# TruongKhang/cds-mvsnet

Hardware: AMD Instinct MI355X
Metric: depth-maps/sec per ref view at 640x512 N=5 D=192 (single-stage plane sweep incl. CostRegNet + regression) (higher is better)
Workload: dtype f32; 1 GPU; M1: single-stage StageNet volume 640x512, D=192, C=8, N=5 views; parallelism=single

## Files before the change

cds_mvsnet_amd/_lib.py:

```python
from __future__ import annotations

import ctypes
import os
from ctypes import c_float, c_int, c_longlong, c_void_p

_HERE = os.path.dirname(os.path.abspath(__file__))
LIB_PATH = os.environ.get("CDS_MVSNET_LIB") or os.path.join(_HERE, "libcdsmvs_hip.so")

ACT_NONE, ACT_RELU, ACT_LEAKY01, ACT_SIGMOID, ACT_TANH = 0, 1, 2, 3, 4
ACT_ACCUM = 16
AGG_ACCUMULATE, AGG_NORMALIZE, AGG_CHANNELS_LAST, AGG_FAST_POSITIONS = 1, 2, 4, 8
WARP_FAST_POSITIONS = AGG_FAST_POSITIONS
MAX_VIEWS = 8
MAX_IMAGES = 16
STAGE_STATE_WORDS = 2080
DEPTH_METRICS_MAX_T = 8
DEPTH_METRICS_MAX_GROUPS = 1024
ICP_SUMS = 18
ICP_MAX_GROUPS = 1024
CROP_MAX_VERTICES = 256
RANSAC_RECORD = 15
RANSAC_MIN_SAMPLE, RANSAC_MAX_SAMPLE = 3, 8
EINVAL = -1000

# ... 13 lines not shown
    "cds_warp_aggregate_f32": [P, P, P, P, P, P, P, I, I, I, I, I, I, I, P],
    "cds_warp_entropy_window_f32": [P, P, P, P, P, I, I, I, I, I, I, I, I, P],
    "cds_warp_aggregate_window_f32": [P, P, P, P, P, P, P, I, I, I, I, I, I, I, I, P],
    "cds_warp_aggregate_bwd_f32": [P, P, P, P, P, P, P, P, P, I, I, I, I, I, I, P],
    "cds_volume_finish_f32": [P, P, P, I, I, I, I, P, P, P],
    "cds_volume_finish_bwd_f32": [P, P, P, P, P, I, I, I, I, P, P, P, P, P],
    "cds_volume_normalize_f32": [P, P, I, I, I, P],
    "cds_volume_normalize_cl_f32": [P, P, I, I, I, P],
    "cds_softargmin_conf_f32": [P, P, P, P, P, I, I, I, I, P],
    "cds_depth_hypotheses_f32": [P, P, I, I, I, I, I, I, P, P, P],
    "cds_depth_planes_f32": [P, I, I, I, P, P],
    "cds_conv3d_k3_f32": [P, P, P, P, P, I, I, I, I, I, I, I, P],
    "cds_conv3d_k3_cl_f32": [P, P, P, P, P, I, I, I, I, I, I, P],
    "cds_conv3d_sbf_f32": [P, P, P, P, P, I, I, I, I, I, I, I, P],
    "cds_conv3d_sf16_f32": [P, P, P, P, I, I, I, I, I, I, I, P, F, P, P],
    "cds_deconv3d_sbf_f32": [P, P, P, P, P, I, I, I, I, I, I, I, P],
    "cds_deconv3d_sf16_f32": [P, P, P, P, P, I, I, I, I, I, I, P, F, P, P],
    "cds_deconv3d_zm_sf16_f32": [P, P, P, P, P, I, I, I, I, I, I, P, F, P, P],
    "cds_deconv_prob_zm_f32": [P, P, P, P, P, P, I, I, I, P],
    "cds_deconv_prob_zm_sf16_f32": [P, P, P, P, P, P, I, I, I, P, F, P],
    "cds_deconv_prob_zm_sf16_mfma_f32": [P, P, P, P, P, P, P, I, I, I, P, F, P, F, F, P],
    "cds_deconv3d_zm_f32": [P, P, P, P, P, I, I, I, I, I, I, P],
    "cds_deconv3d_k3s2_f32": [P, P, P, P, P, I, I, I, I, I, I, P],
    "cds_conv2d_f32": [P, P, P, P, I, I, I, I, I, I, I, I, I, P],
    "cds_conv2d_affine_f32": [P, P, P, P, P, I, I, I, I, I, I, I, I, I, P],
    "cds_instnorm_affine_f32": [P, P, P, I, I, I, I, F, P],
    "cds_fpn_stats_parts": [I, I],
    "cds_conv2d_fpn_f32": [P, P, P, P, P, P, P, I, I, I, I, I, I, P],
    "cds_conv2d_k3_c16_f32": [P, P, P, P, P, P, I, I, I, I, P],
    "cds_dynconv_branches_sbf_f32": [P, P, P, P, P, I, I, I, I, I, P, I, P],
    "cds_dynconv_fused_sbf_f32": [P, P, P, P, P, P, P, P, F, P, P, P, I, I, I, I, I, P, I, P],
    "cds_dynconv_fused_parts": [I, I],
    "cds_conv2d_k3_relu_sbf_f32": [P, P, P, P, P, P, I, I, I, I, P],
    "cds_dynconv_blend_f32": [P, P, P, P, P, F, P, P, I, I, I, I, I, P],
    "cds_dynconv_blend_shared_f32": [P, P, P, P, P, F, P, P, I, I, I, I, I, I, P],
    "cds_blend_stats_parts": [I, I],
    "cds_dynconv_blend_stats_f32": [P, P, P, P, P, F, P, P, P, I, I, I, I, I, I, P],
    "cds_instnorm_reduce_f32": [P, I, P, P, I, I, I, I, F, P],
    "cds_instnorm_apply_f32": [P, P, P, I, I, I, I, I, I, P],
    "cds_instnorm_act_f32": [P, P, P, I, I, I, I, I, I, P],
    "cds_debug_poison_lds": [ctypes.c_uint],
    "cds_dynconv_cl_parts": [I, I],
    "cds_dynconv_cl_f32": [P, P, P, P, P, P, P, P, F, P, P, P, I, I, I, I, P, I, P],
    "cds_dynconv_cl_sf16_f32": [P, P, P, P, P, P, P, P, F, P, P, P, I, I, I, I, P, I, F, F, P],
    "cds_conv00_cl_f32": [P, P, P, P, P, P, P, F, P, P, P, I, I, I, I, P],
    "cds_conv00_cl_sf16_f32": [P, P, P, P, P, P, P, F, P, P, P, I, I, I, I, P, F, P],
    "cds_blend_cl_parts": [I, I],
    "cds_dynconv_blend_cl_f32": [P, P, P, P, P, F, P, P, P, I, I, I, I, I, I, P],
    "cds_conv2d_k3s2_cl_f32": [P, P, P, P, I, I, I, I, I, P],
    "cds_conv2d_k3s2_cl_sf16_f32": [P, P, P, P, I, I, I, I, I, F, F, P],
    "cds_fpn_cl_parts": [I, I],
    "cds_conv2d_fpn_cl_f32": [P, P, P, P, P, P, P, I, I, I, I, I, I, P],
    "cds_vis_layer1_cl_f32": [P, P, P, P, P, I, I, I, P],
    "cds_conv2d_k3_relu_cl_f32": [P, P, P, P, P, P, I, I, I, I, P],
    "cds_instnorm_stats_cl_parts": [I, I],
    "cds_instnorm_stats_cl_f32": [P, P, I, I, I, I, P],
    "cds_instnorm_apply_cl_f32": [P, P, P, P, I, I, I, I, I, I, I, P],
    "cds_curvature_stats_f32": [P, P, P, P, P, I, P],
    "cds_curvature_stats_bwd_f32": [P, P, P, P, P, P, P, P, I, P],
    "cds_pair_mean_f32": [P, P, I, I, P],
    "cds_view_mean_f32": [P, P, I, I, P],
    "cds_depth_affine_f32": [P, P, I, P, P],
    "cds_deconv2d_k3s2_f32": [P, P, P, P, I, I, I, I, I, P],
    "cds_refine_finish_f32": [P, P, P, I, I, P, P],
    "cds_bn3d_stats_f32": [P, P, I, I, L, P],
    "cds_bn3d_norm_f32": [P, P, P, P, DB, DB, F, P, P, P, P, P, P, P, P, I, I, L, I, P],
    "cds_bn3d_bwd_reduce_f32": [P, P, P, P, P, I, I, L, I, P],
    "cds_bn3d_bwd_norm_f32": [P, P, P, P, P, P, P, DB, P, P, P, I, I, L, I, P],
    "cds_conv3d_wgrad_f32": [P, P, P, I, I, I, I, I, I, I, I, I, I, P],
    "cds_bn3d_norm_bound_f32": [P, P, P, P, DB, DB, F, P, P, P, P, P, P, P, P, I, I, L, I, P, P],
    "cds_bn3d_bwd_norm_bound_f32": [P, P, P, P, P, P, P, DB, P, P, P, I, I, L, I, P, P],
    "cds_absmax_bound_f32": [P, L, P, P],
    "cds_sf16_pack_conv3d_f32": [P, P, P, P, I, I, I, P],
    "cds_conv3d_k3_sf16_f32": [P, P, P, P, P, I, I, I, I, I, I, I, P],
    "cds_conv3d_wgrad_sf16_f32": [P, P, P, P, P, I, I, I, I, I, I, I, I, I, I, P],
    "cds_conv2d_wgrad_f32": [P, P, P, I, I, I, I, I, I, I, I, I, I, P],
    "cds_conv2d_dgrad_s2_f32": [P, P, P, I, I, I, I, I, I, I, P],
    "cds_instnorm_bwd_f32": [P, P, P, P, P, I, I, I, I, I, I, P],
    "cds_dynconv_bn_stats_f32": [P, P, P, P, P, P, P, P, I, I, I, I, I, I, F, F, I, I, P],
    "cds_dynconv_blend_train_f32": [P, P, P, P, P, P, P, P, F, P, P, I, I, I, I, I, I, P],
    "cds_dynconv_blend_bwd_f32": [P, P, P, P, P, P, P, P, F, P, P, P, P, P, I, I, I, I, I, I, I, I, P],
    "cds_f32_to_bf16": [P, P, L, P],
    "cds_instnorm_act_b16_f32": [P, P, P, P, P, I, I, I, I, I, I, P],
    "cds_conv2d_wgrad_xb16_f32": [P, P, P, I, I, I, I, I, I, I, I, I, I, P],
    "cds_instnorm_bwd_yb16_f32": [P, P, P, P, P, P, I, I, I, I, I, I, P],
    "cds_dynconv_bn_stats_b16_f32": [P, P, P, P, P, P, P, P, I, I, I, I, I, I, F, F, I, I, P],
    "cds_dynconv_blend_train_b16_f32": [P, P, P, P, P, P, P, P, F, P, P, I, I, I, I, I, I, P],
    "cds_dynconv_blend_bwd_b16_f32": [P, P, P, P, P, P, P, P, F, P, P, P, P, P, I, I, I, I, I, I, I, I, P],
    "cds_pack_conv2d_f32": [P, P, P, P, I, I, I, I, P],
    "cds_pack_conv3d_f32": [P, P, P, I, I, I, P],
    "cds_softargmin_bwd_f32": [P, P, P, P, I, I, I, I, P],
    "cds_dynconv_bwd_finish_f32": [P, P, I, I, P, P],
    "cds_bn_running_update_f32": [P, P, P, F, I, I, P, P, P],
    "cds_loss_records": [ctypes.c_longlong],
    "cds_loss_stage_f32": [P, P, P, P, P, P, P, I, I, I, P, P, P],
    "cds_loss_final_f32": [P, P, P, P, P, P, I, P, P, P, P],
    "cds_loss_stage_bwd_f32": [P, P, P, P, P, P, P, P, F, I, I, I, P, P, P, P],
    "cds_feat_target_f32": [P, P, P, F, F, I, I, I, P, P],
    "cds_depth_fusion_f32": [P, P, P, P, P, P, P, P, P, I, I, I, P, F, F, F, P],
    "cds_depth_fusion_dynamic_f32": [P, P, P, P, P, P, P, P, P, P, I, I, I, P, F, F, I, I, P],
    "cds_depth_normals_f32": [P, P, P, I, I, I, F, I, P, P, P],
    "cds_voxel_merge_f32": [P, P, P, L, P, P, L, P, P, P, P, P],
    "cds_tsdf_integrate_f32": [P, L, P, P, DB, P, P, P, P, I, I, I, P, P, P, P, P],
    "cds_tsdf_integrate_w_f32": [P, L, P, P, DB, P, P, P, P, I, I, I, P, P, P, P, P, I, F, P, P],
    "cds_tsdf_view_weights": [P, P, P, P, P, P, I, I, P, P],
    "cds_tsdf_classify": [P, P, L, P, P, P, P, I, P, P, P, P, P],
# ... 89 lines not shown
```

cds_mvsnet_amd/csrc/feat_cl.hip:

```cpp
#include "sbf_common.hpp"
#include "feat_common.hpp"

namespace {

constexpr int TX = 32, TY = 8;

struct DynEpi {
  const float* w1;
  const float* b1;
  const float* w2;
  float* out;
  float* norm_curv;
  double* partial;
  float temperature;
  const float* epi;
  float xs, omul;
};

constexpr int cmax(int a, int b) { return a > b ? a : b; }
constexpr int nks_of(int k) { return (k * k + 3) / 4; }

template <int CIN, int K0, int K1, int K2, int MODE = 1>
struct DCfg {
  static constexpr int NBR = MODE == 2 ? 1 : (K2 > 0 ? 3 : 2);
// ... 1022 lines not shown
      const int ky = tap / 3, kx = tap - ky * 3;
      const unsigned char* ap = lp + ((2 * wave + ky) * IXP + 2 * m + kx) * POSB;
      BV wh[NBLK], wlo[NBLK], ah[2], alo[2];
#pragma unroll
      for (int nb = 0; nb < NBLK; ++nb) {
        const uint4* p = wr + (size_t)((t * NBLK + nb) * 3) * 64;
        wh[nb].u = p[0];
        wlo[nb].u = p[64];
      }
#pragma unroll
      for (int q = 0; q < 2; ++q) {
        const unsigned char* a = ap + q * 32 * POSB;
        ah[q].u = *reinterpret_cast<const uint4*>(a);
        alo[q].u = *reinterpret_cast<const uint4*>(a + 16);
      }
      __builtin_amdgcn_sched_barrier(0);
#pragma unroll
      for (int nb = 0; nb < NBLK; ++nb) {
#pragma unroll
        for (int q = 0; q < 2; ++q) SF16_MFMA(acc[nb][q], alo[q], wh[nb]);
#pragma unroll
        for (int q = 0; q < 2; ++q) SF16_MFMA(acc[nb][q], ah[q], wlo[nb]);
#pragma unroll
        for (int q = 0; q < 2; ++q) SF16_MFMA(acc[nb][q], ah[q], wh[nb]);
      }
    }
  }
  __syncthreads();
  float* trL = reinterpret_cast<float*>(lds) + wave * (2 * NBLK * 16 * C::TP);
#pragma unroll
  for (int nb = 0; nb < NBLK; ++nb)
#pragma unroll
    for (int q = 0; q < 2; ++q) {
      const f32x4 a = acc[nb][q] * omul;
      const float v[4] = {a.x, a.y, a.z, a.w};
#pragma unroll
      for (int i = 0; i < 4; ++i) trL[((q * NBLK + nb) * 16 + g * 4 + i) * C::TP + m] = v[i];
    }
  wave_lds_fence();
  const int oy = oy0 + wave;
  if (oy < Ho) {
#pragma unroll
    for (int q = 0; q < 2; ++q) {
      const int ox = ox0 + q * 16 + m;
      if (ox >= Wo) continue;
      float* __restrict__ op = out + (((size_t)img * Ho + oy) * Wo + ox) * COUT;
#pragma unroll
      for (int nb = 0; nb < NBLK; ++nb)
        *reinterpret_cast<float4*>(op + nb * 16 + 4 * g) = *reinterpret_cast<const float4*>(trL + ((q * NBLK + nb) * 16 + m) * C::TP + 4 * g);
    }
  }
}

}

extern "C" int cds_vis_layer1_cl_f32(const float* entropy, const float* ref_nc, const float* weight, const float* bias, float* out, int V,
                                     int H, int W, void* stream) {
  if (!entropy || !ref_nc || !weight || !bias || !out || V < 1 || H < 1 || W < 1) return CDS_EINVAL;
  hipLaunchKernelGGL(vis_layer1_cl_kernel, dim3(cds_ceil_div(H * W, 256), V), dim3(256), 0, (hipStream_t)stream, entropy, ref_nc, weight,
                     bias, out, H, W);
  return cds_launch_status();
}

extern "C" int cds_conv2d_k3_relu_cl_f32(const float* x, const void* weight_split, const float* bias, const float* head_w,
                                         const float* head_b, float* out, int N, int Cin, int H, int W, void* stream) {
  if (!x || !weight_split || !out || N < 1 || Cin != 16 || H < 1 || W < 1 || (head_w != nullptr) != (head_b != nullptr)) return CDS_EINVAL;
  DynEpi ep{};
  ep.w1 = head_w;
  ep.b1 = head_b;
  ep.out = out;
  return launch_dynconv_cl<16, 3, 0, 0, 2>(x, nullptr, weight_split, bias, ep, N, H, W, (hipStream_t)stream);
}

extern "C" int cds_dynconv_cl_parts(int H, int W) { return cds_ceil_div(W, TX) * cds_ceil_div(H, TY); }

extern "C" int cds_dynconv_cl_f32(const float* x, const float* in_affine, const void* weight_split, const float* bias,
                                  const float* w1, const float* b1, const float* w2, const float* epipoles, float temperature,
                                  float* out, float* norm_curv, double* partial, int N, int C, int H, int W, const int* ksizes, int nb,
                                  void* stream) {
  if (!x || !weight_split || !w1 || !b1 || !w2 || !epipoles || !out || !norm_curv || !partial || !ksizes || N < 1 ||
      N > CDS_MAX_IMAGES || H < 1 || W < 1 || nb < 2 || nb > 3)
    return CDS_EINVAL;
  DynEpi ep{};
  ep.w1 = w1; ep.b1 = b1; ep.w2 = w2; ep.out = out; ep.norm_curv = norm_curv; ep.partial = partial; ep.temperature = temperature;
  ep.epi = epipoles;
  hipStream_t st = (hipStream_t)stream;
  const int k0 = ksizes[0], k1 = ksizes[1], k2 = nb == 3 ? ksizes[2] : 0;
  if (C == 8 && k0 == 3 && k1 == 5 && k2 == 7) return launch_dynconv_cl<8, 3, 5, 7>(x, in_affine, weight_split, bias, ep, N, H, W, st);
  if (C == 8 && k0 == 1 && k1 == 3 && k2 == 0) return launch_dynconv_cl<8, 1, 3, 0>(x, in_affine, weight_split, bias, ep, N, H, W, st);
  if (C == 16 && k0 == 3 && k1 == 5 && k2 == 0) return launch_dynconv_cl<16, 3, 5, 0>(x, in_affine, weight_split, bias, ep, N, H, W, st);
  if (C == 16 && k0 == 1 && k1 == 3 && k2 == 0) return launch_dynconv_cl<16, 1, 3, 0>(x, in_affine, weight_split, bias, ep, N, H, W, st);
  if (C == 32 && k0 == 1 && k1 == 3 && k2 == 0) return launch_dynconv_cl<32, 1, 3, 0>(x, in_affine, weight_split, bias, ep, N, H, W, st);
  return CDS_EINVAL;
}

extern "C" int cds_dynconv_cl_sf16_f32(const float* x, const float* in_affine, const void* weight_split, const float* bias,
                                       const float* w1, const float* b1, const float* w2, const float* epipoles, float temperature,
                                       float* out, float* norm_curv, double* partial, int N, int C, int H, int W, const int* ksizes,
                                       int nb, float x_bound, float w_inv_scale, void* stream) {
  if (!x || !weight_split || !w1 || !b1 || !w2 || !epipoles || !out || !norm_curv || !partial || !ksizes || N < 1 ||
      N > CDS_MAX_IMAGES || H < 1 || W < 1 || nb < 2 || nb > 3 || !(x_bound > 0.f) || !(w_inv_scale > 0.f))
    return CDS_EINVAL;
  DynEpi ep{};
  ep.w1 = w1; ep.b1 = b1; ep.w2 = w2; ep.out = out; ep.norm_curv = norm_curv; ep.partial = partial; ep.temperature = temperature;
  ep.epi = epipoles;
  int e = 0;
  (void)frexpf(x_bound, &e);
  e = e > 100 ? 100 : (e < -100 ? -100 : e);
  ep.xs = ldexpf(1.0f, 15 - e);
  ep.omul = w_inv_scale / ep.xs;
  hipStream_t st = (hipStream_t)stream;
  const int k0 = ksizes[0], k1 = ksizes[1], k2 = nb == 3 ? ksizes[2] : 0;
  if (C == 8 && k0 == 3 && k1 == 5 && k2 == 7) return launch_dynconv_cl<8, 3, 5, 7, 1, true>(x, in_affine, weight_split, bias, ep, N, H, W, st);
  if (C == 8 && k0 == 1 && k1 == 3 && k2 == 0) return launch_dynconv_cl<8, 1, 3, 0, 1, true>(x, in_affine, weight_split, bias, ep, N, H, W, st);
  if (C == 16 && k0 == 3 && k1 == 5 && k2 == 0) return launch_dynconv_cl<16, 3, 5, 0, 1, true>(x, in_affine, weight_split, bias, ep, N, H, W, st);
  if (C == 16 && k0 == 1 && k1 == 3 && k2 == 0) return launch_dynconv_cl<16, 1, 3, 0, 1, true>(x, in_affine, weight_split, bias, ep, N, H, W, st);
  if (C == 32 && k0 == 1 && k1 == 3 && k2 == 0) return launch_dynconv_cl<32, 1, 3, 0, 1, true>(x, in_affine, weight_split, bias, ep, N, H, W, st);
  return CDS_EINVAL;
}

static int conv00_entry(const float* x, const void* weight_split, const float* bias, const float* w1, const float* b1, const float* w2,
                        const float* epipoles, float temperature, float* out, float* norm_curv, double* partial, int N, int n_shared,
                        int H, int W, const float* in_bound, float w_inv_scale, void* stream) {
  if (!x || !weight_split || !w1 || !b1 || !w2 || !epipoles || !out || !norm_curv || !partial || N < 1 || N > CDS_MAX_IMAGES ||
// ... 145 lines not shown
```

cds_mvsnet_amd/csrc/lib.hip:

```cpp
#include "cds_common.hpp"
extern "C" int cds_version(void) { return 100;  }

namespace {
__global__ __launch_bounds__(1024) void poison_lds_kernel(unsigned pattern, int words) {
  extern __shared__ unsigned lds_words[];
  for (int i = threadIdx.x; i < words; i += 1024) lds_words[i] = pattern;
}
}

extern "C" int cds_debug_poison_lds(unsigned pattern) {
  const int bytes = 160 * 1024;
  static std::atomic<unsigned long long> ok{0};
  if (int e = cds_allow_lds(reinterpret_cast<const void*>(poison_lds_kernel), bytes, ok)) return e;
  if (hipDeviceSynchronize() != hipSuccess) return -1;
  hipLaunchKernelGGL(poison_lds_kernel, dim3(2048), dim3(1024), bytes, 0, pattern, bytes / 4);
  if (hipDeviceSynchronize() != hipSuccess) return -1;
  return 0;
}
```

cds_mvsnet_amd/model.py:

```python
from __future__ import annotations

import os
import weakref
from typing import Dict, List, Optional, Sequence, Tuple

import torch
import torch.nn as nn
import torch.nn.functional as F

from . import geometry, ops
from .ops import ACT_LEAKY01, ACT_NONE, ACT_RELU, ACT_SIGMOID, ACT_TANH

Tensor = torch.Tensor
BN_EPS = 1e-5
USE_SPLIT_BF16 = os.environ.get("CDS_CONV_EXACT", "0") != "1"
USE_FUSED_BLEND = os.environ.get("CDS_FUSED_BLEND", "1") != "0"
OVERLAP_STAGE1 = os.environ.get("CDS_OVERLAP_STAGE1", "1") != "0"
OVERLAP_STAGE2 = os.environ.get("CDS_OVERLAP_STAGE2", "0") == "1"
USE_FEAT_CL = os.environ.get("CDS_FEAT_CL", "1") != "0"
USE_CONV00_MFMA = os.environ.get("CDS_CONV00_MFMA", "1") != "0"
OVERLAP_IN_CAPTURE = os.environ.get("CDS_OVERLAP_IN_CAPTURE", "1") != "0"
_SIDE_STREAMS: Dict[int, "torch.cuda.Stream"] = {}
USE_GRAPHS_DEFAULT = os.environ.get("CDS_GRAPH", "0") == "1"
_GRAPH_RUNNERS: "weakref.WeakKeyDictionary" = weakref.WeakKeyDictionary()


_UNIT_BOUNDS: Dict[int, Tensor] = {}


def _unit_bound(device) -> Tensor:
    idx = device.index if device.index is not None else torch.cuda.current_device()
    if idx not in _UNIT_BOUNDS:
        _UNIT_BOUNDS[idx] = torch.ones((1,), dtype=torch.float32, device=device)
    return _UNIT_BOUNDS[idx]


def _side_stream(device) -> "torch.cuda.Stream":
    idx = device.index if device.index is not None else torch.cuda.current_device()
    if idx not in _SIDE_STREAMS:
        _SIDE_STREAMS[idx] = torch.cuda.Stream(device=device)
    return _SIDE_STREAMS[idx]


def _bn_fold(bn: nn.Module) -> Tuple[Tensor, Tensor]:
    scale = bn.weight.detach() / torch.sqrt(bn.running_var + bn.eps)
    shift = bn.bias.detach() - bn.running_mean * scale
    return scale, shift


def _pack2d(w: Tensor) -> Tensor:
    cout, cin, k, _ = w.shape
    p = w.permute(1, 2, 3, 0).reshape(cin, k * k, cout)
    pad = (-cout) % 8
    if pad:
        p = F.pad(p, (0, pad))
    return p.contiguous()


class _Packed:

    def __init__(self):
        self._entries: Dict[object, Tuple[tuple, Dict[str, Tensor]]] = {}
        self.generation = 0

    def invalidate(self) -> None:
        self._entries = {}
        self.generation += 1

    @staticmethod
    def _tensors(owner: nn.Module) -> List[Tensor]:
        return list(owner.parameters()) + list(owner.buffers())

    def get(self, owner: nn.Module, builder) -> Dict[str, Tensor]:
# ... 534 lines not shown
            return self._conv00(x[0])
        p = self.p
        w, kw = self._operand(name, *x)
        return ops.dynconv_cl(x[0], w, p.get(f"{name}.bs"), dc.size_kernels, p[f"{name}.m1"], p[f"{name}.mb"], p[f"{name}.m2"],
                              self.epi[level], self.T, 0.1, in_affine=x[1], **kw)

    def down(self, name: str, x):
        w, kw = self._operand(name, *x, plain=".w9")
        y = ops.conv2d_k3s2_cl(x[0], None if kw else w, getattr(self.net, name).conv.out_channels, x[1], wsplit=w if kw else None, **kw)
        return y, ops.instnorm_stats_cl(y, 0.1)[1]

    def lateral(self, name: str, coarse, skip):
        return ops.conv2d_fpn_cl(coarse[0], skip[0], self.p[f"{name}.wt"], getattr(self.net, name).conv.out_channels, coarse[1], skip[1], 0.1)

    def head(self, name: str, x, level: int, stage: int):
        o, nc, st, _ = self._dynconv(name, getattr(self.net, name), x, level)
        n = self.n_chw
        if stage == 2:
            on, chw = ops.instnorm_apply_cl(o, st, ACT_TANH, n, cl_from=0)
            return (chw, on[n:] if n < o.shape[0] else None), (on, None), nc
        hwc, chw = ops.instnorm_apply_cl(o, st, ACT_TANH, n, cl_from=n)
        return (chw, hwc), None, nc


class StageNet(_PackedHolder):
    def __init__(self, num_mvs_stages: int = 3):
        super().__init__()
        self.vis = nn.ModuleList([nn.Sequential(ConvBn2d(2, 16), ConvBn2d(16, 16), ConvBn2d(16, 16),
                                                nn.Conv2d(16, 1, 1), nn.Sigmoid()) for _ in range(num_mvs_stages)])
        self._init_packed()

    def _pack(self) -> Dict[str, Tensor]:
        out: Dict[str, Tensor] = {}
        for s, seq in enumerate(self.vis):
            for i in range(3):
                scale, shift = _bn_fold(seq[i].bn)
                wf = seq[i].conv.weight.detach() * scale.view(-1, 1, 1, 1)
                out[f"{s}.w{i}"] = _pack2d(wf)
                out[f"{s}.b{i}"] = shift.contiguous()
                if i > 0:
                    out[f"{s}.wcl{i}"] = wf.permute(2, 3, 0, 1).reshape(9, 16, 16).contiguous()
                    if USE_SPLIT_BF16 and wf.is_cuda:
                        out[f"{s}.ws{i}"] = ops.split_pack_dynconv([wf])
            out[f"{s}.w3"] = _pack2d(seq[3].weight.detach())
            out[f"{s}.b3"] = seq[3].bias.detach().contiguous()
            out[f"{s}.hw"] = seq[3].weight.detach().reshape(16).contiguous()
        return out

    def visibility(self, entropy: Tensor, ref_nc: Tensor, stage_idx: int) -> Tensor:
        p = self._packed.get(self, self._pack)
        s = stage_idx
        with ops.prof("visibility_cnn"):
            if USE_FEAT_CL and f"{s}.ws1" in p and ops.USE_CONV2D_SBF:
                x = ops.vis_layer1_cl(entropy.contiguous(), ref_nc.contiguous(), p[f"{s}.w0"], p[f"{s}.b0"])
                x = ops.conv2d_k3_relu_cl(x, p[f"{s}.ws1"], p[f"{s}.b1"])
                return ops.conv2d_k3_relu_cl(x, p[f"{s}.ws2"], p[f"{s}.b2"], head_w=p[f"{s}.hw"], head_b=p[f"{s}.b3"])
            x = torch.stack((entropy, ref_nc), dim=1)
            x = ops.conv2d(x, p[f"{s}.w0"], p[f"{s}.b0"], 16, 3, 1, 1, ACT_RELU)
            if f"{s}.ws1" in p and ops.USE_CONV2D_SBF and x.shape[-1] % 4 == 0:
                x = ops.conv2d_k3_relu_sbf(x, p[f"{s}.ws1"], p[f"{s}.b1"])
                return ops.conv2d_k3_relu_sbf(x, p[f"{s}.ws2"], p[f"{s}.b2"], head_w=p[f"{s}.hw"], head_b=p[f"{s}.b3"])
            if ops.conv2d_c16_supported(x):
                x = ops.conv2d_k3_c16(x, p[f"{s}.wcl1"], p[f"{s}.b1"], ACT_RELU)
                return ops.conv2d_k3_c16(x, p[f"{s}.wcl2"], p[f"{s}.b2"], ACT_RELU, head_w=p[f"{s}.hw"], head_b=p[f"{s}.b3"])
            for i in (1, 2):
                x = ops.conv2d(x, p[f"{s}.w{i}"], p[f"{s}.b{i}"], 16, 3, 1, 1, ACT_RELU)
            return ops.conv2d(x, p[f"{s}.w3"], p[f"{s}.b3"], 1, 1, 1, 0, ACT_SIGMOID)[:, 0]

    def aggregate(self, ref_chw: Tensor, src_hwc: Tensor, ref_nc: Tensor, mats: Tensor, hyp: Tensor, stage_idx: int,
                  normalize: bool = True, channels_last: bool = False):
        ent = ops.warp_entropy(ref_chw, src_hwc, mats, hyp)
        vis = self.visibility(ent, ref_nc, stage_idx).contiguous()
        volume, vis_sum = ops.warp_aggregate(ref_chw, src_hwc, vis, mats, hyp, normalize=normalize, channels_last=channels_last)
        return volume, vis_sum, ent, vis

    def run_single(self, ref_chw, src_hwc, ref_nc, nc_sums, mats, hyp, cost_regularization, stage_idx, vol_bound=None, nc_mean=None):
        cl = isinstance(cost_regularization, CostRegNet) and cost_regularization.split_bf16_supported()
        volume, _, _, _ = self.aggregate(ref_chw, src_hwc, ref_nc, mats, hyp, stage_idx, channels_last=cl)
        if cl:
            if vol_bound is None and ops.USE_SPLIT_F16:
                vol_bound = (ref_chw.abs().amax() * src_hwc.abs().amax()).reshape(1)
            depth, conf = cost_regularization.regress(volume, hyp, bound=vol_bound)
        else:
            depth, conf = ops.softargmin_conf(cost_regularization(volume), hyp)
        del volume
        if nc_mean is None:
            nc_mean = ops.view_mean(nc_sums.contiguous())
        return depth, conf, nc_mean

    def forward(self, features, proj_matrices, depth_values, num_depth, cost_regularization, prob_volume_init=None,
                stage_idx=0, gt_depth=None):
        if prob_volume_init is not None:
            raise NotImplementedError("prob_volume_init is dead code in the reference (never passed)")
        assert len(features) == proj_matrices.shape[1] - 1, "Different number of images and projection matrices"
        assert depth_values.shape[1] == num_depth, f"depth_values.shape[1]:{depth_values.shape[1]}  num_depth:{num_depth}"
        if self.training or gt_depth is not None:
            from .training import stage_forward_train
            dv = depth_values
            if dv.dim() == 2:
                h, w = features[0]["ref"][0].shape[-2:]
                dv = dv.view(*dv.shape, 1, 1).expand(-1, -1, h, w)
            with torch.cuda.device(dv.device):
                return stage_forward_train(self, features, proj_matrices, dv, cost_regularization, stage_idx, gt_depth)
        with torch.cuda.device(depth_values.device):
            return self._forward(features, proj_matrices, depth_values, cost_regularization, stage_idx)

# ... 267 lines not shown
```

cds_mvsnet_amd/ops.py:

```python
from __future__ import annotations

import ctypes
import os
from typing import Optional, Tuple

import torch

from . import _lib
from ._lib import (ACT_LEAKY01, ACT_NONE, ACT_RELU, ACT_SIGMOID, ACT_TANH, AGG_ACCUMULATE, AGG_CHANNELS_LAST, AGG_FAST_POSITIONS,
                   AGG_NORMALIZE,
                   MAX_IMAGES, MAX_VIEWS, check)

Tensor = torch.Tensor

PROFILE_ON = False
PROFILE: dict = {}
PROFILE_HOST_MS: dict = {}


class prof:

    def __init__(self, name: str):
        self.name = name
        self.start = None
# ... 1100 lines not shown
    check(lib.cds_conv2d_fpn_cl_f32(_dev(coarse_cl, "coarse"), _dev(coarse_affine, "coarse_affine") if coarse_affine is not None else None,
                                    _dev(skip_cl, "skip"), _dev(skip_affine, "skip_affine") if skip_affine is not None else None,
                                    _dev(w, "weight"), out.data_ptr(), partial.data_ptr() if partial is not None else None,
                                    N, Ca, Cb, cout, H, W, _stream(skip_cl)), "cds_conv2d_fpn_cl_f32")
    if stats_slope is None:
        return out
    return out, _reduce_records(partial, N, cout, H, W, stats_slope)[1]


def instnorm_apply_cl(x_cl: Tensor, stats: Tensor, act: int, n_chw: int = 0, cl_from: Optional[int] = 0):
    N, H, W, C = x_cl.shape
    if stats.dtype != torch.float64 or tuple(stats.shape) != (N, C, 2):
        raise ValueError(f"instnorm_apply_cl: stats must be float64 [{N},{C},2]")
    want_cl = cl_from is not None and cl_from < N
    if not want_cl and n_chw < 1:
        raise ValueError("instnorm_apply_cl: nothing to write")
    dev = x_cl.device
    out_cl = torch.empty((N - cl_from, H, W, C), dtype=torch.float32, device=dev) if want_cl else None
    out_chw = torch.empty((n_chw, C, H, W), dtype=torch.float32, device=dev) if n_chw > 0 else None
    check(_lib.load().cds_instnorm_apply_cl_f32(_dev(x_cl, "x"), _dev64(stats, "stats"), out_cl.data_ptr() if want_cl else None,
                                                out_chw.data_ptr() if n_chw > 0 else None, N, C, H, W, act, n_chw,
                                                cl_from if want_cl else 0, _stream(x_cl)), "cds_instnorm_apply_cl_f32")
    return out_cl, out_chw


def vis_layer1_cl(entropy: Tensor, ref_nc: Tensor, wpk: Tensor, bias: Tensor) -> Tensor:
    V, h, w = entropy.shape
    if tuple(ref_nc.shape) != (V, h, w) or tuple(wpk.shape) != (2, 9, 16) or bias.numel() != 16:
        raise ValueError(f"vis_layer1_cl: need entropy / ref_nc [V,h,w], weight [2,9,16], bias [16]; got {tuple(entropy.shape)}, "
                         f"{tuple(ref_nc.shape)}, {tuple(wpk.shape)}")
    out = torch.empty((V, h, w, 16), dtype=torch.float32, device=entropy.device)
    check(_lib.load().cds_vis_layer1_cl_f32(_dev(entropy, "entropy"), _dev(ref_nc, "ref_nc"), _dev(wpk, "weight"), _dev(bias, "bias"),
                                            out.data_ptr(), V, h, w, _stream(entropy)), "cds_vis_layer1_cl_f32")
    return out


def conv2d_k3_relu_cl(x_cl: Tensor, wsplit: Tensor, bias: Optional[Tensor], head_w: Optional[Tensor] = None,
                      head_b: Optional[Tensor] = None) -> Tensor:
    N, H, W, C = x_cl.shape
    if C != 16:
        raise ValueError(f"conv2d_k3_relu_cl: need [N,H,W,16], got {tuple(x_cl.shape)}")
    if (head_w is None) != (head_b is None) or (head_w is not None and (head_w.numel() != 16 or head_b.numel() != 1)):
        raise ValueError("conv2d_k3_relu_cl: head_w [16] and head_b [1] go together")
    if wsplit.dtype != torch.int16 or wsplit.numel() != 2 * 3 * 1 * 3 * 64 * 8:
        raise ValueError("conv2d_k3_relu_cl: wsplit must be split_pack_dynconv([w]) of a [16,16,3,3] weight")
    out = torch.empty((N, H, W) if head_w is not None else (N, H, W, 16), dtype=torch.float32, device=x_cl.device)
    check(_lib.load().cds_conv2d_k3_relu_cl_f32(_dev(x_cl, "x"), wsplit.data_ptr(), _dev(bias, "bias") if bias is not None else None,
                                                _dev(head_w, "head_w") if head_w is not None else None,
                                                _dev(head_b, "head_b") if head_b is not None else None,
                                                out.data_ptr(), N, C, H, W, _stream(x_cl)), "cds_conv2d_k3_relu_cl_f32")
    return out


def depth_fusion(ref_depth: Tensor, ref_conf: Tensor, src_depths: Tensor, src_confs: Tensor, cams: Tensor,
                 prob_thresh, dist_thresh: float, depth_thresh: float, view_thresh: float,
                 want_view_masks: bool = False):
    V, h, w = src_depths.shape
    if tuple(ref_depth.shape) != (h, w) or tuple(ref_conf.shape) != (3, h, w) or tuple(src_confs.shape) != (V, 3, h, w) \
            or tuple(cams.shape) != (V, 100):
        raise ValueError("depth_fusion: inconsistent shapes")
    dev = ref_depth.device
    fused = torch.empty((h, w), dtype=torch.float32, device=dev)
    mask = torch.empty((h, w), dtype=torch.float32, device=dev)
    points = torch.empty((3, h, w), dtype=torch.float32, device=dev)
    vm = torch.empty((V, h, w), dtype=torch.float32, device=dev) if want_view_masks else None
    th = torch.tensor([float(p) for p in prob_thresh], dtype=torch.float32)
    if th.numel() != 3:
        raise ValueError("depth_fusion: three confidence thresholds expected")
    check(_lib.load().cds_depth_fusion_f32(_dev(ref_depth, "ref_depth"), _dev(ref_conf, "ref_conf"),
                                           _dev(src_depths, "src_depths"), _dev(src_confs, "src_confs"),
                                           _dev(cams, "cams"), fused.data_ptr(), mask.data_ptr(), points.data_ptr(),
                                           vm.data_ptr() if vm is not None else None, V, h, w, _host(th, "prob_thresh"),
                                           float(dist_thresh), float(depth_thresh), float(view_thresh),
                                           _stream(fused)), "cds_depth_fusion_f32")
    return fused, mask, points, vm


DYNAMIC_MAX_LEVELS = 16


def depth_fusion_dynamic(ref_depth: Tensor, ref_conf: Tensor, src_depths: Tensor, src_confs: Tensor, cams: Tensor,
                         prob_thresh, dist_base: float = 0.25, rel_base: float = 1.0 / 1300.0, n_views=(2, 10),
                         want_admit: bool = False, want_levels: bool = False):
    V, h, w = src_depths.shape
    if tuple(ref_depth.shape) != (h, w) or tuple(ref_conf.shape) != (3, h, w) or tuple(src_confs.shape) != (V, 3, h, w) \
            or tuple(cams.shape) != (V, 100):
        raise ValueError("depth_fusion_dynamic: inconsistent shapes")
    if len(n_views) != 2:
        raise ValueError(f"depth_fusion_dynamic: n_views must be (n_min, n_max), got {n_views!r}")
    n_min, n_max = int(n_views[0]), int(n_views[1])
    if n_min < 1 or n_max < n_min or n_max > DYNAMIC_MAX_LEVELS:
        raise ValueError(f"depth_fusion_dynamic: need 1 <= n_min <= n_max <= {DYNAMIC_MAX_LEVELS}, got {(n_min, n_max)}")
    if not (float(dist_base) > 0.0 and float(rel_base) > 0.0):
        raise ValueError(f"depth_fusion_dynamic: dist_base and rel_base must be positive, got {dist_base}, {rel_base}")
    th = torch.tensor([float(p) for p in prob_thresh], dtype=torch.float32)
    if th.numel() != 3:
        raise ValueError("depth_fusion_dynamic: three confidence thresholds expected")
    dev = ref_depth.device
    fused = torch.empty((h, w), dtype=torch.float32, device=dev)
    mask = torch.empty((h, w), dtype=torch.float32, device=dev)
    points = torch.empty((3, h, w), dtype=torch.float32, device=dev)
    admit = torch.empty((h, w), dtype=torch.uint8, device=dev) if want_admit else None
    levels = torch.empty((V, h, w), dtype=torch.uint8, device=dev) if want_levels else None
    check(_lib.load().cds_depth_fusion_dynamic_f32(_dev(ref_depth, "ref_depth"), _dev(ref_conf, "ref_conf"),
                                                   _dev(src_depths, "src_depths"), _dev(src_confs, "src_confs"),
                                                   _dev(cams, "cams"), fused.data_ptr(), mask.data_ptr(), points.data_ptr(),
# ... 449 lines not shown
```

include/cds_mvsnet_hip.h:

```cpp
#ifndef CDS_MVSNET_HIP_H
#define CDS_MVSNET_HIP_H

#ifdef __cplusplus
extern "C" {
#endif

#define CDS_EINVAL (-1000)
#define CDS_MAX_VIEWS 8
#define CDS_MAX_IMAGES 16
#define CDS_STAGE_STATE_WORDS 2080

#define CDS_ACT_NONE 0
#define CDS_ACT_RELU 1
#define CDS_ACT_LEAKY01 2
#define CDS_ACT_SIGMOID 3
#define CDS_ACT_ACCUM 16
#define CDS_ACT_TANH 4

#define CDS_AGG_ACCUMULATE 1
#define CDS_AGG_NORMALIZE 2
#define CDS_AGG_CHANNELS_LAST 4
#define CDS_AGG_FAST_POSITIONS 8
#define CDS_WARP_FAST_POSITIONS CDS_AGG_FAST_POSITIONS

// ... 117 lines not shown
int cds_dynconv_blend_shared_f32(const float* branches, const float* w1, const float* b1, const float* w2,
                                 const float* epipoles, float temperature, float* out, float* norm_curv, int N,
                                 int K, int Cout, int H, int W, int n_shared, void* stream);

int cds_blend_stats_parts(int H, int W);
int cds_dynconv_blend_stats_f32(const float* branches, const float* w1, const float* b1, const float* w2,
                                const float* epipoles, float temperature, float* out, float* norm_curv,
                                float* partial, int N, int K, int Cout, int H, int W, int n_shared, void* stream);
int cds_instnorm_reduce_f32(const float* partial, int parts, float* stats, float* affine, int N, int C, int H, int W,
                            float slope, void* stream);
int cds_instnorm_apply_f32(const float* x, const float* stats, float* out, int N, int C, int H, int W, int act,
                           int out_hwc, void* stream);

int cds_instnorm_act_f32(const float* x, float* out, float* stats, int N, int C, int H, int W, int act,
                         int out_hwc, void* stream);
int cds_instnorm_affine_f32(const float* x, float* affine, float* stats, int N, int C, int H, int W, float slope,
                            void* stream);

int cds_debug_poison_lds(unsigned pattern);

int cds_dynconv_cl_parts(int H, int W);
int cds_dynconv_cl_f32(const float* x, const float* in_affine, const void* weight_split, const float* bias, const float* w1,
                       const float* b1, const float* w2, const float* epipoles, float temperature, float* out,
                       float* norm_curv, double* partial, int N, int C, int H, int W, const int* ksizes, int nb, void* stream);
int cds_dynconv_cl_sf16_f32(const float* x, const float* in_affine, const void* weight_split, const float* bias, const float* w1,
                            const float* b1, const float* w2, const float* epipoles, float temperature, float* out, float* norm_curv,
                            double* partial, int N, int C, int H, int W, const int* ksizes, int nb, float x_bound, float w_inv_scale,
                            void* stream);

int cds_conv00_cl_f32(const float* x, const void* weight_split, const float* bias, const float* w1, const float* b1, const float* w2,
                      const float* epipoles, float temperature, float* out, float* norm_curv, double* partial, int N, int n_shared,
                      int H, int W, void* stream);
int cds_conv00_cl_sf16_f32(const float* x, const void* weight_split, const float* bias, const float* w1, const float* b1, const float* w2,
                           const float* epipoles, float temperature, float* out, float* norm_curv, double* partial, int N, int n_shared,
                           int H, int W, const float* in_bound, float w_inv_scale, void* stream);

int cds_blend_cl_parts(int H, int W);
int cds_dynconv_blend_cl_f32(const float* branches, const float* w1, const float* b1, const float* w2, const float* epipoles,
                             float temperature, float* out, float* norm_curv, double* partial, int N, int K, int Cout, int H, int W,
                             int n_shared, void* stream);
int cds_conv2d_k3s2_cl_f32(const float* x, const float* in_affine, const float* weight, float* out, int N, int Cin, int Cout, int H,
                           int W, void* stream);
int cds_conv2d_k3s2_cl_sf16_f32(const float* x, const float* in_affine, const void* weight_split, float* out, int N, int Cin, int Cout,
                                int H, int W, float x_bound, float w_inv_scale, void* stream);

int cds_fpn_cl_parts(int H, int W);
int cds_conv2d_fpn_cl_f32(const float* coarse, const float* coarse_affine, const float* skip, const float* skip_affine,
                          const float* weight, float* out, double* partial, int N, int Ca, int Cb, int Cout, int H, int W,
                          void* stream);
int cds_vis_layer1_cl_f32(const float* entropy, const float* ref_nc, const float* weight, const float* bias, float* out, int V, int H,
                          int W, void* stream);
int cds_conv2d_k3_relu_cl_f32(const float* x, const void* weight_split, const float* bias, const float* head_w, const float* head_b,
                              float* out, int N, int Cin, int H, int W, void* stream);
int cds_instnorm_stats_cl_parts(int H, int W);
int cds_instnorm_stats_cl_f32(const float* x, double* partial, int N, int C, int H, int W, void* stream);
int cds_instnorm_apply_cl_f32(const float* x, const double* stats, float* out_cl, float* out_chw, int N, int C, int H, int W, int act,
                              int n_chw, int cl_from, void* stream);

int cds_depth_fusion_f32(const float* ref_depth, const float* ref_conf, const float* src_depths,
                         const float* src_confs, const float* cams, float* fused, float* mask, float* points,
                         float* view_masks, int V, int h, int w, const float* prob_thresh_host,
                         float dist_thresh, float depth_thresh, float view_thresh, void* stream);

int cds_depth_fusion_dynamic_f32(const float* ref_depth, const float* ref_conf, const float* src_depths,
                                 const float* src_confs, const float* cams, float* fused, float* mask, float* points,
                                 unsigned char* admit, unsigned char* levels, int V, int h, int w,
                                 const float* prob_thresh_host, float dist_base, float rel_base, int n_min, int n_max,
                                 void* stream);

int cds_depth_normals_f32(const float* depth, const unsigned char* valid, const float* cam_host, int h, int w, int radius,
                          float jump, int min_pts, float* normals, unsigned char* ok, void* stream);

int cds_voxel_merge_f32(const float* points, const unsigned* colors, const float* normals, long long n, const long long* perm,
                        const int* start, long long n_voxels, float* out_points, unsigned* out_colors, float* out_normals,
                        int* out_counts, void* stream);

#define CDS_TSDF_MAX_CHUNK 32
#define CDS_TSDF_MAX_CELLS (1 << 26)
int cds_tsdf_integrate_f32(const int* keys, long long n_blocks, const double* frame_host, const int* dims_host, double trunc,
                           const float* depths, const unsigned char* masks, const unsigned char* images, const double* cams,
                           int n_views, int h, int w, float* sum, int* n, int* nc, int* rgb, void* stream);
int cds_tsdf_classify(const int* keys, const int* table, long long n_blocks, const double* frame_host, const int* dims_host,
                      const float* sum, const int* n, int min_weight, unsigned char* vmask, unsigned char* tcount,
                      int* block_vertices, int* block_faces, void* stream);
int cds_tsdf_emit(const int* keys, const int* table, long long n_blocks, const double* frame_host, const int* dims_host,
                  const float* sum, const int* n, const int* nc, const int* rgb, const unsigned char* vmask,
                  const unsigned char* tcount, const int* block_vstart, const int* block_tstart, long long n_vertices,
                  long long n_faces, int* vstart, float* vertices, unsigned char* colors, int* faces, void* stream);

int cds_tsdf_view_weights(const float* depth, const unsigned char* mask, const float* normals, const unsigned char* ok,
                          const float* conf, const float* cam_host, int h, int w, unsigned char* weights, void* stream);
int cds_tsdf_integrate_w_f32(const int* keys, long long n_blocks, const double* frame_host, const int* dims_host, double trunc,
                             const float* depths, const unsigned char* masks, const unsigned char* images, const double* cams,
                             int n_views, int h, int w, float* sum, int* n, int* nc, int* rgb, const unsigned char* weights,
                             int interp, float jump, int* wn, void* stream);

#define CDS_RASTER_CAM 24
#define CDS_RASTER_MAX_CHUNK 32
#define CDS_RASTER_MAX_LIST (1ll << 30)
int cds_raster_project(const float* vertices, long long n_vertices, const double* cams, int n_views, int* xy, double* xc,
                       void* stream);
int cds_raster_faces(const int* faces, long long n_faces, long long n_vertices, const double* cams, int n_views, const int* xy,
                     const double* xc, int h, int w, long long large_px, unsigned long long* keys, unsigned char* large,
                     void* stream);
int cds_raster_large(const long long* list, long long n_list, const int* faces, long long n_faces, long long n_vertices,
                     const double* cams, int n_views, const int* xy, const double* xc, int h, int w, unsigned long long* keys,
// ... 224 lines not shown
```

Before: 189.8 depth-maps/s.

## Fuse three-layer visibility CNN into one tiled kernel with LDS halos

Measured after the change: 187.0 depth-maps/s. -1.4%, worse.

```diff
diff --git a/cds_mvsnet_amd/_lib.py b/cds_mvsnet_amd/_lib.py
--- a/cds_mvsnet_amd/_lib.py
+++ b/cds_mvsnet_amd/_lib.py
@@ -89,6 +89,7 @@
     "cds_fpn_cl_parts": [I, I],
     "cds_conv2d_fpn_cl_f32": [P, P, P, P, P, P, P, I, I, I, I, I, I, P],
     "cds_vis_layer1_cl_f32": [P, P, P, P, P, I, I, I, P],
+    "cds_vis_cnn_cl_f32": [P, P, P, P, P, P, P, P, P, P, P, I, I, I, P],
     "cds_conv2d_k3_relu_cl_f32": [P, P, P, P, P, P, I, I, I, I, P],
     "cds_instnorm_stats_cl_parts": [I, I],
     "cds_instnorm_stats_cl_f32": [P, P, I, I, I, I, P],
diff --git a/cds_mvsnet_amd/csrc/feat_cl.hip b/cds_mvsnet_amd/csrc/feat_cl.hip
--- a/cds_mvsnet_amd/csrc/feat_cl.hip
+++ b/cds_mvsnet_amd/csrc/feat_cl.hip
@@ -1098,6 +1098,188 @@
   }
 }
 
+struct VisF {
+  static constexpr int OX = 30, OY = 8;
+  static constexpr int X2 = OX + 2, Y2 = OY + 2, N2 = X2 * Y2;
+  static constexpr int X1 = OX + 4, Y1 = OY + 4, N1 = X1 * Y1;
+  static constexpr int X0 = OX + 6, Y0 = OY + 6, N0 = X0 * Y0;
+  static constexpr int PL1 = N1 * POSB, PL2 = N2 * POSB;
+  static constexpr int OFF2 = 2 * PL1, OFFT = OFF2 + 2 * PL2;
+  static constexpr int TP = 20;
+  static constexpr int LDSB = OFFT + 4 * 16 * TP * 4;
+  static constexpr int T2 = Y2 * 2 / 4, T3 = OY * 2 / 4;
+};
+static_assert(VisF::X2 == 32 && VisF::Y2 * 2 % 4 == 0, "layer-2 region: two 16-pixel runs per row, whole N-tiles per wave");
+static_assert(2 * VisF::N0 * 4 <= 2 * VisF::PL2, "the input maps are staged where the layer-2 region will be");
+
+__device__ __forceinline__ void vis_load_weights(BV (&w)[6][3], const uint4* __restrict__ wl) {
+#pragma unroll
+  for (int s = 0; s < 6; ++s)
+#pragma unroll
+    for (int term = 0; term < 3; ++term) w[s][term].u = wl[(s * 3 + term) * 64];
+}
+
+template <int NT, int PITCH, int PLANE>
+__device__ __forceinline__ void vis_kloop(f32x4 (&acc)[NT], const unsigned char* __restrict__ region, const int (&off)[NT],
+                                          const BV (&w)[6][3], int m, int g) {
+#pragma unroll
+  for (int s = 0; s < 6; ++s) {
+    const int rd = s / 3, t = s - rd * 3;
+    int tap = 4 * t + g;
+    if (tap > 8) tap = 8;
+    const int ky = tap / 3, kx = tap - ky * 3;
+    const unsigned char* ap = region + rd * PLANE + (ky * PITCH + kx + m) * POSB;
+    BV ah[NT], am[NT], al[NT];
+#pragma unroll
+    for (int q = 0; q < NT; ++q) {
+      const unsigned char* a = ap + off[q];
+      al[q].u = *reinterpret_cast<const uint4*>(a + 32);
+      am[q].u = *reinterpret_cast<const uint4*>(a + 16);
+      ah[q].u = *reinterpret_cast<const uint4*>(a);
+    }
+    __builtin_amdgcn_sched_barrier(0);
+#pragma unroll
+    for (int q = 0; q < NT; ++q) SBF_MFMA(acc[q], al[q], w[s][0]);
+#pragma unroll
+    for (int q = 0; q < NT; ++q) SBF_MFMA(acc[q], am[q], w[s][1]);
+#pragma unroll
+    for (int q = 0; q < NT; ++q) SBF_MFMA(acc[q], ah[q], w[s][2]);
+#pragma unroll
+    for (int q = 0; q < NT; ++q) SBF_MFMA(acc[q], am[q], w[s][0]);
+#pragma unroll
+    for (int q = 0; q < NT; ++q) SBF_MFMA(acc[q], ah[q], w[s][1]);
+#pragma unroll
+    for (int q = 0; q < NT; ++q) SBF_MFMA(acc[q], ah[q], w[s][0]);
+    __builtin_amdgcn_sched_barrier(0);
+  }
+}
+
+__global__ __launch_bounds__(256, 2) void vis_cnn_cl_kernel(const float* __restrict__ ent, const float* __restrict__ nc,
+                                                            const float* __restrict__ w0, const float* __restrict__ b0,
+                                                            const uint4* __restrict__ ws1, const float* __restrict__ b1,
+                                                            const uint4* __restrict__ ws2, const float* __restrict__ b2,
+                                                            const float* __restrict__ head_w, const float* __restrict__ head_b,
+                                                            float* __restrict__ out, int V, int H, int W, int tiles_x, int tiles_y) {
+  using C = VisF;
+  extern __shared__ __attribute__((aligned(16))) unsigned char lds[];
+  int lin = cds_xcd_remap(blockIdx.x, tiles_x * tiles_y * V);
+  const int tx_i = lin % tiles_x;
+  lin /= tiles_x;
+  const int ty_i = lin % tiles_y, img = lin / tiles_y;
+  const int tid = threadIdx.x, lane = tid & 63;
+  const int wave = __builtin_amdgcn_readfirstlane(tid >> 6);
+  const int m = lane & 15, g = lane >> 4;
+  const int ox0 = tx_i * C::OX, oy0 = ty_i * C::OY;
+
+  float* in0 = reinterpret_cast<float*>(lds + C::OFF2);
+  {
+    const float* __restrict__ e = ent + (size_t)img * H * W;
+    const float* __restrict__ n = nc + (size_t)img * H * W;
+    for (int p = tid; p < C::N0; p += 256) {
+      const int row = p / C::X0, col = p - row * C::X0;
+      const int gy = oy0 - 3 + row, gx = ox0 - 3 + col;
+      const bool ok = (unsigned)gy < (unsigned)H && (unsigned)gx < (unsigned)W;
+      in0[p] = ok ? e[(size_t)gy * W + gx] : 0.f;
+      in0[C::N0 + p] = ok ? n[(size_t)gy * W + gx] : 0.f;
+    }
+  }
+  BV w[6][3];
+  vis_load_weights(w, ws1 + lane);
+  const float bv1 = b1[m], bv2 = b2[m], hw_n = head_w[m], hb = head_b[0];
+  __syncthreads();
+
+  for (int pos = tid; pos < C::N1; pos += 256) {
+    const int row = pos / C::X1, col = pos - row * C::X1;
+    const int gy = oy0 - 2 + row, gx = ox0 - 2 + col;
+    float o[16];
+#pragma unroll
+    for (int c = 0; c < 16; ++c) o[c] = 0.f;
+    if ((unsigned)gy < (unsigned)H && (unsigned)gx < (unsigned)W) {
+      float acc[16];
+#pragma unroll
+      for (int c = 0; c < 16; ++c) acc[c] = 0.f;
+#pragma unroll
+      for (int ci = 0; ci < 2; ++ci)
+#pragma unroll
+        for (int ky = 0; ky < 3; ++ky)
+#pragma unroll
+          for (int kx = 0; kx < 3; ++kx) {
+            const float v = in0[ci * C::N0 + (row + ky) * C::X0 + col + kx];
+            const float* __restrict__ wc = w0 + (ci * 9 + ky * 3 + kx) * 16;
+#pragma unroll
+            for (int c = 0; c < 16; ++c) acc[c] = fmaf(v, wc[c], acc[c]);
+          }
+#pragma unroll
+      for (int c = 0; c < 16; ++c) o[c] = fmaxf(acc[c] + b0[c], 0.f);
+    }
+    unsigned char* d = lds + pos * POSB;
+    split_store8(d, make_float4(o[0], o[1], o[2], o[3]), make_float4(o[4], o[5], o[6], o[7]));
+    split_store8(d + C::PL1, make_float4(o[8], o[9], o[10], o[11]), make_float4(o[12], o[13], o[14], o[15]));
+  }
+  __syncthreads();
+
+  {
+    f32x4 acc[C::T2];
+    int off[C::T2];
+#pragma unroll
+    for (int i = 0; i < C::T2; ++i) {
+      const int j = wave + 4 * i;
+      acc[i] = (f32x4){0.f, 0.f, 0.f, 0.f};
+      off[i] = ((j >> 1) * C::X1 + (j & 1) * 16) * POSB;
+    }
+    vis_kloop<C::T2, C::X1, C::PL1>(acc, lds, off, w, m, g);
+    vis_load_weights(w, ws2 + lane);
+    const float bv = bv1;
+    float* trL = reinterpret_cast<float*>(lds + C::OFFT) + wave * (16 * C::TP);
+    unsigned char* dst0 = lds + C::OFF2 + (g >> 1) * C::PL2 + (g & 1) * 8;
+#pragma unroll
+    for (int i = 0; i < C::T2; ++i) {
+      const f32x4 a = acc[i];
+      const float v[4] = {fmaxf(a.x + bv, 0.f), fmaxf(a.y + bv, 0.f), fmaxf(a.z + bv, 0.f), fmaxf(a.w + bv, 0.f)};
+#pragma unroll
+      for (int k = 0; k < 4; ++k) trL[(g * 4 + k) * C::TP + m] = v[k];
+      wave_lds_fence();
+      float4 t = *reinterpret_cast<const float4*>(trL + m * C::TP + 4 * g);
+      wave_lds_fence();
+      const int j = wave + 4 * i;
+      const int row = j >> 1, col = (j & 1) * 16 + m;
+      const int gy = oy0 - 1 + row, gx = ox0 - 1 + col;
+      if (!((unsigned)gy < (unsigned)H && (unsigned)gx < (unsigned)W)) t = make_float4(0.f, 0.f, 0.f, 0.f);
+      uint32_t h0, m0, l0, h1, m1, l1;
+      split2(t.x, t.y, h0, m0, l0);
+      split2(t.z, t.w, h1, m1, l1);
+      unsigned char* d = dst0 + (row * C::X2 + col) * POSB;
+      *reinterpret_cast<uint2*>(d) = make_uint2(h0, h1);
+      *reinterpret_cast<uint2*>(d + 16) = make_uint2(m0, m1);
+      *reinterpret_cast<uint2*>(d + 32) = make_uint2(l0, l1);
+    }
+  }
+  __syncthreads();
+
+  f32x4 acc[C::T3];
+  int off[C::T3];
+#pragma unroll
+  for (int q = 0; q < C::T3; ++q) {
+    acc[q] = (f32x4){0.f, 0.f, 0.f, 0.f};
+    off[q] = ((wave * 2 + (q >> 1)) * C::X2 + (q & 1) * 14) * POSB;
+  }
+  vis_kloop<C::T3, C::X2, C::PL2>(acc, lds + C::OFF2, off, w, m, g);
+  const float bv = bv2;
+#pragma unroll
+  for (int q = 0; q < C::T3; ++q) {
+    const int px0 = (q & 1) * 14 + g * 4;
+    const int oy = oy0 + wave * 2 + (q >> 1), ox = ox0 + px0;
+    const f32x4 a = acc[q];
+    float v[4] = {fmaxf(a.x + bv, 0.f), fmaxf(a.y + bv, 0.f), fmaxf(a.z + bv, 0.f), fmaxf(a.w + bv, 0.f)};
+#pragma unroll
+    for (int i = 0; i < 4; ++i) v[i] = row16_sum(v[i] * hw_n) + hb;
+    const int i = m & 3;
+    const float sacc = i == 0 ? v[0] : i == 1 ? v[1] : i == 2 ? v[2] : v[3];
+    const float vis = 1.0f / (1.0f + expf(-sacc));
+    if (m < 4 && oy < H && ox + i < W && px0 + i >= (q & 1) * 16) out[((size_t)img * H + oy) * W + ox + i] = vis;
+  }
+}
+
 }
 
 extern "C" int cds_vis_layer1_cl_f32(const float* entropy, const float* ref_nc, const float* weight, const float* bias, float* out, int V,
@@ -1116,6 +1298,19 @@
   ep.b1 = head_b;
   ep.out = out;
   return launch_dynconv_cl<16, 3, 0, 0, 2>(x, nullptr, weight_split, bias, ep, N, H, W, (hipStream_t)stream);
+}
+
+extern "C" int cds_vis_cnn_cl_f32(const float* entropy, const float* ref_nc, const float* w0, const float* b0, const void* ws1,
+                                  const float* b1, const void* ws2, const float* b2, const float* head_w, const float* head_b, float* out,
+                                  int V, int H, int W, void* stream) {
+  if (!entropy || !ref_nc || !w0 || !b0 || !ws1 || !b1 || !ws2 || !b2 || !head_w || !head_b || !out || V < 1 || H < 1 || W < 1)
+    return CDS_EINVAL;
+  static std::atomic<unsigned long long> lds_ok{0};
+  if (int e = cds_allow_lds(reinterpret_cast<const void*>(vis_cnn_cl_kernel), VisF::LDSB, lds_ok)) return e;
+  const int tx = cds_ceil_div(W, VisF::OX), ty = cds_ceil_div(H, VisF::OY);
+  hipLaunchKernelGGL(vis_cnn_cl_kernel, dim3(tx * ty * V), dim3(256), (size_t)VisF::LDSB, (hipStream_t)stream, entropy, ref_nc, w0, b0,
+                     reinterpret_cast<const uint4*>(ws1), b1, reinterpret_cast<const uint4*>(ws2), b2, head_w, head_b, out, V, H, W, tx, ty);
+  return cds_launch_status();
 }
 
 extern "C" int cds_dynconv_cl_parts(int H, int W) { return cds_ceil_div(W, TX) * cds_ceil_div(H, TY); }
diff --git a/cds_mvsnet_amd/csrc/lib.hip b/cds_mvsnet_amd/csrc/lib.hip
--- a/cds_mvsnet_amd/csrc/lib.hip
+++ b/cds_mvsnet_amd/csrc/lib.hip
@@ -1,5 +1,5 @@
 #include "cds_common.hpp"
-extern "C" int cds_version(void) { return 100;  }
+extern "C" int cds_version(void) { return 101;  }
 
 namespace {
 __global__ __launch_bounds__(1024) void poison_lds_kernel(unsigned pattern, int words) {
diff --git a/cds_mvsnet_amd/model.py b/cds_mvsnet_amd/model.py
--- a/cds_mvsnet_amd/model.py
+++ b/cds_mvsnet_amd/model.py
@@ -18,7 +18,8 @@
 OVERLAP_STAGE1 = os.environ.get("CDS_OVERLAP_STAGE1", "1") != "0"
 OVERLAP_STAGE2 = os.environ.get("CDS_OVERLAP_STAGE2", "0") == "1"
 USE_FEAT_CL = os.environ.get("CDS_FEAT_CL", "1") != "0"
-USE_CONV00_MFMA = os.environ.get("CDS_CONV00_MFMA", "1") != "0"
+USE_VIS_FUSED = os.environ.get("CDS_VIS_FUSED", "1") != "0"
+USE_CONV00_MFMA =os.environ.get("CDS_CONV00_MFMA", "1") != "0"
 OVERLAP_IN_CAPTURE = os.environ.get("CDS_OVERLAP_IN_CAPTURE", "1") != "0"
 _SIDE_STREAMS: Dict[int, "torch.cuda.Stream"] = {}
 USE_GRAPHS_DEFAULT = os.environ.get("CDS_GRAPH", "0") == "1"
@@ -659,6 +660,9 @@
         s = stage_idx
         with ops.prof("visibility_cnn"):
             if USE_FEAT_CL and f"{s}.ws1" in p and ops.USE_CONV2D_SBF:
+                if USE_VIS_FUSED:
+                    return ops.vis_cnn_cl(entropy.contiguous(), ref_nc.contiguous(), p[f"{s}.w0"], p[f"{s}.b0"], p[f"{s}.ws1"], p[f"{s}.b1"],
+                                          p[f"{s}.ws2"], p[f"{s}.b2"], p[f"{s}.hw"], p[f"{s}.b3"])
                 x = ops.vis_layer1_cl(entropy.contiguous(), ref_nc.contiguous(), p[f"{s}.w0"], p[f"{s}.b0"])
                 x = ops.conv2d_k3_relu_cl(x, p[f"{s}.ws1"], p[f"{s}.b1"])
                 return ops.conv2d_k3_relu_cl(x, p[f"{s}.ws2"], p[f"{s}.b2"], head_w=p[f"{s}.hw"], head_b=p[f"{s}.b3"])
diff --git a/cds_mvsnet_amd/ops.py b/cds_mvsnet_amd/ops.py
--- a/cds_mvsnet_amd/ops.py
+++ b/cds_mvsnet_amd/ops.py
@@ -1176,6 +1176,28 @@
     return out
 
 
+VIS_CNN_CL_LAUNCHES = 0
+
+
+def vis_cnn_cl(entropy: Tensor, ref_nc: Tensor, w0: Tensor, b0: Tensor, ws1: Tensor, b1: Tensor, ws2: Tensor, b2: Tensor,
+               head_w: Tensor, head_b: Tensor) -> Tensor:
+    global VIS_CNN_CL_LAUNCHES
+    V, h, w = entropy.shape
+    if tuple(ref_nc.shape) != (V, h, w) or tuple(w0.shape) != (2, 9, 16) or any(b.numel() != 16 for b in (b0, b1, b2, head_w)) \
+            or head_b.numel() != 1:
+        raise ValueError(f"vis_cnn_cl: need entropy / ref_nc [V,h,w], w0 [2,9,16], b0 / b1 / b2 / head_w [16], head_b [1]; got "
+                         f"{tuple(entropy.shape)}, {tuple(ref_nc.shape)}, {tuple(w0.shape)}")
+    for ws in (ws1, ws2):
+        if ws.dtype != torch.int16 or ws.numel() != 2 * 3 * 1 * 3 * 64 * 8 or not ws.is_cuda:
+            raise ValueError("vis_cnn_cl: ws1 / ws2 must be split_pack_dynconv([w]) of a [16,16,3,3] weight")
+    out = torch.empty((V, h, w), dtype=torch.float32, device=entropy.device)
+    check(_lib.load().cds_vis_cnn_cl_f32(_dev(entropy, "entropy"), _dev(ref_nc, "ref_nc"), _dev(w0, "w0"), _dev(b0, "b0"), ws1.data_ptr(),
+                                         _dev(b1, "b1"), ws2.data_ptr(), _dev(b2, "b2"), _dev(head_w, "head_w"), _dev(head_b, "head_b"),
+                                         out.data_ptr(), V, h, w, _stream(entropy)), "cds_vis_cnn_cl_f32")
+    VIS_CNN_CL_LAUNCHES += 1
+    return out
+
+
 def depth_fusion(ref_depth: Tensor, ref_conf: Tensor, src_depths: Tensor, src_confs: Tensor, cams: Tensor,
                  prob_thresh, dist_thresh: float, depth_thresh: float, view_thresh: float,
                  want_view_masks: bool = False):
diff --git a/include/cds_mvsnet_hip.h b/include/cds_mvsnet_hip.h
--- a/include/cds_mvsnet_hip.h
+++ b/include/cds_mvsnet_hip.h
@@ -193,6 +193,9 @@
                           int W, void* stream);
 int cds_conv2d_k3_relu_cl_f32(const float* x, const void* weight_split, const float* bias, const float* head_w, const float* head_b,
                               float* out, int N, int Cin, int H, int W, void* stream);
+int cds_vis_cnn_cl_f32(const float* entropy, const float* ref_nc, const float* w0, const float* b0, const void* ws1, const float* b1,
+                       const void* ws2, const float* b2, const float* head_w, const float* head_b, float* out, int V, int H, int W,
+                       void* stream);
 int cds_instnorm_stats_cl_parts(int H, int W);
 int cds_instnorm_stats_cl_f32(const float* x, double* partial, int N, int C, int H, int W, void* stream);
 int cds_instnorm_apply_cl_f32(const float* x, const double* stats, float* out_cl, float* out_chw, int N, int C, int H, int W, int act,
```
